# imdea-software/legosnark

Measured on AMD Instinct MI355X. Metric: alt_bn128 G1 MSM point-scalar pairs/s at n=2^20, higher is better.
Workload: dtype u32 limbs (254-bit Montgomery integers)

## Files before the change

legosnark_amd/csrc/curves.h:

```cpp
#pragma once
#include "ec.h"
#include "fp29.h"
#include "fp29x2.h"
#include "quad29.h"

namespace lsa {

struct CurveG1 {
    using Field = Fq;
    using Base = AffPacked;
    using Acc = XYZZ29;
    static constexpr bool GLV = true;
    static __device__ __forceinline__ Acc inf() { return Acc::inf(); }
    static __device__ __forceinline__ Acc madd(const Acc &a, const Base &b, bool negate, bool endo) {
        Aff29 q = unpack_affine(b);
        if (q.is_inf()) return a;
        if (negate) q.y = sub_k<1>(F29::zero(), q.y);
        if (endo) {
            constexpr uint32_t BETA29[9] = {0x0a337995u, 0x158d1d23u, 0x189c9b98u, 0x12fa4e45u, 0x185faadcu,
                                            0x0176f16du, 0x0eed93bau, 0x14291140u, 0x000c0afeu};
            q.x = mul(q.x, F29::from_limbs(BETA29));
        }
        return xyzz29_madd(a, q);
    }
    static __device__ __forceinline__ Acc add(const Acc &a, const Acc &b) { return xyzz29_add(a, b); }
    static __device__ __forceinline__ Acc dbl(const Acc &a) { return xyzz29_dbl(a); }
    static __device__ __forceinline__ Jac<Fq> to_jac(const Acc &a) { return xyzz29_to_jac(a); }
    static __device__ __forceinline__ Acc from_jac(const Jac<Fq> &p) {
        if (p.Z.is_zero()) return Acc::inf();
        F29 z = F29::from_mont256(p.Z), zz = sqr(z);
        return {F29::from_mont256(p.X), F29::from_mont256(p.Y), zz, mul(zz, z)};
    }
    static __device__ __forceinline__ Base from_affine(const Aff<Fq> &a) {
        Base r;
        if (a.is_inf()) {
#pragma unroll
            for (int i = 0; i < 8; i++) { r.x[i] = 0; r.y[i] = 0; }
        } else {
            F29::from_mont256(a.x).canonical().pack256(r.x);
            F29::from_mont256(a.y).canonical().pack256(r.y);
        }
        return r;
    }
};
struct CurveG2 {
    using Field = Fq2;
    using Base = AffPackedG2;
    using Acc = XYZZ29x2;
    static constexpr bool GLV = false;
    static __device__ __forceinline__ Acc inf() { return Acc::inf(); }
    static __device__ __forceinline__ Acc madd(const Acc &a, const Base &b, bool negate, bool ) {
        Aff29x2 q = unpack_affine(b);
        if (q.is_inf()) return a;
        if (negate) q.y = sub_k<1>(F29x2::zero(), q.y);
        return g2_madd(a, q);
    }
    static __device__ __forceinline__ Acc add(const Acc &a, const Acc &b) { return g2_add(a, b); }
    static __device__ __forceinline__ Acc dbl(const Acc &a) { return g2_dbl(a); }
    static __device__ __forceinline__ Jac<Fq2> to_jac(const Acc &a) { return g2_to_jac(a); }
    static __device__ __forceinline__ Acc from_jac(const Jac<Fq2> &p) {
        if (p.Z.is_zero()) return Acc::inf();
        F29x2 z = f29x2_from_mont256(p.Z), zz = sqr<2>(z);
        return {f29x2_from_mont256(p.X), f29x2_from_mont256(p.Y), zz, mul<2>(zz, z)};
    }
    static __device__ __forceinline__ Base from_affine(const Aff<Fq2> &a) { return pack_affine_g2(a); }
};
template <class F> struct CurveOf;
template <> struct CurveOf<Fq> { using type = CurveG1; };
template <> struct CurveOf<Fq2> { using type = CurveG2; };


}
```

legosnark_amd/csrc/fp29.h:

```cpp
#pragma once
#include "ec.h"

namespace lsa {

LSA_HD uint32_t lsa_mask(uint32_t m) {
#if defined(__HIP_DEVICE_COMPILE__)
    asm volatile("" : "+v"(m));
#endif
    return m;
}

struct F29 {
    static constexpr int W = 29;
    static constexpr uint32_t MASK = (1u << 29) - 1;
    static constexpr uint32_t PINV = 0x04866389u;
    static constexpr uint32_t PINV_POS = 0x1b799c77u;
    uint32_t l[9];

    static LSA_HD uint32_t p(int i) {
        constexpr uint32_t P29[9] = {0x187cfd47u, 0x010460b6u, 0x1c72a34fu, 0x02d522d0u, 0x1585d978u,
                                     0x02db40c0u, 0x00a6e141u, 0x0e5c2634u, 0x0030644eu};
        return P29[i];
    }
    static LSA_HD F29 from_limbs(const uint32_t (&c)[9]) {
// ... 32 lines not shown
        r.l[8] = (uint32_t)((int32_t)l[8] + c);
        return r;
    }

    friend LSA_HD F29 add_lazy(const F29 &a, const F29 &b) {
        F29 r;
#pragma unroll
        for (int i = 0; i < 9; i++) r.l[i] = a.l[i] + b.l[i];
        return r;
    }
    template <int K>
    friend LSA_HD F29 sub_k(const F29 &a, const F29 &b);

    static LSA_HD F29 redc_cols(uint64_t (&col)[17]) {
        uint64_t carry = 0;
        F29 r;
#pragma unroll
        for (int k = 0; k < 9; k++) {
            uint64_t acc = col[k] + carry;
            const uint32_t m = ((uint32_t)acc * PINV) & MASK;
            acc += (uint64_t)m * p(0);
            carry = acc >> 29;
#pragma unroll
            for (int j = 1; j < 9; j++) col[k + j] += (uint64_t)m * p(j);
        }
#pragma unroll
        for (int k = 9; k < 17; k++) {
            const uint64_t acc = col[k] + carry;
            r.l[k - 9] = (uint32_t)acc & MASK;
            carry = acc >> 29;
        }
        r.l[8] = (uint32_t)carry;
        return r;
    }
    friend LSA_HD F29 mul(const F29 &a, const F29 &b) {
#if defined(LSA_FP29_COLS)
        {
            uint64_t col[17];
#pragma unroll
            for (int k = 0; k < 17; k++) col[k] = 0;
#pragma unroll
            for (int i = 0; i < 9; i++)
#pragma unroll
                for (int j = 0; j < 9; j++) col[i + j] += (uint64_t)a.l[i] * b.l[j];
            return redc_cols(col);
        }
#endif
        uint64_t acc = 0;
        uint32_t m[9];
        F29 r;
#pragma unroll
        for (int k = 0; k < 9; k++) {
#pragma unroll
            for (int i = 0; i <= k; i++) acc += (uint64_t)a.l[i] * b.l[k - i];
#pragma unroll
            for (int i = 0; i < k; i++) acc += (uint64_t)m[i] * p(k - i);
            m[k] = ((uint32_t)acc * PINV) & MASK;
            acc += (uint64_t)m[k] * p(0);
            acc >>= 29;
        }
#pragma unroll
        for (int k = 9; k < 17; k++) {
#pragma unroll
            for (int i = k - 8; i < 9; i++) acc += (uint64_t)a.l[i] * b.l[k - i];
#pragma unroll
            for (int i = k - 8; i < 9; i++) acc += (uint64_t)m[i] * p(k - i);
            r.l[k - 9] = (uint32_t)acc & MASK;
            acc >>= 29;
        }
        r.l[8] = (uint32_t)acc;
        return r;
    }
    friend LSA_HD F29 sqr(const F29 &a) {
        uint32_t d[9];
#pragma unroll
        for (int i = 0; i < 9; i++) d[i] = a.l[i] << 1;
#if defined(LSA_FP29_COLS)
        {
            uint64_t col[17];
#pragma unroll
            for (int k = 0; k < 17; k++) col[k] = 0;
#pragma unroll
            for (int i = 0; i < 9; i++) {
                col[2 * i] += (uint64_t)a.l[i] * a.l[i];
#pragma unroll
                for (int j = i + 1; j < 9; j++) col[i + j] += (uint64_t)a.l[i] * d[j];
            }
            return redc_cols(col);
        }
#endif
        uint64_t acc = 0;
        uint32_t m[9];
        F29 r;
#pragma unroll
        for (int k = 0; k < 17; k++) {
#pragma unroll
            for (int i = 0; i < 9; i++) {
                const int j = k - i;
                if (j > i && j < 9) acc += (uint64_t)a.l[i] * d[j];
            }
            if ((k & 1) == 0) acc += (uint64_t)a.l[k / 2] * a.l[k / 2];
            if (k < 9) {
#pragma unroll
                for (int i = 0; i < k; i++) acc += (uint64_t)m[i] * p(k - i);
                m[k] = ((uint32_t)acc * PINV) & MASK;
                acc += (uint64_t)m[k] * p(0);
            } else {
#pragma unroll
                for (int i = k - 8; i < 9; i++) acc += (uint64_t)m[i] * p(k - i);
                r.l[k - 9] = (uint32_t)acc & MASK;
            }
            acc >>= 29;
        }
        r.l[8] = (uint32_t)acc;
        return r;
    }
    friend LSA_HD F29 dot2(const F29 &a0, const F29 &b0, const F29 &a1, const F29 &b1) {
#if defined(LSA_FP29_COLS)
        {
            uint64_t col[17];
#pragma unroll
            for (int k = 0; k < 17; k++) col[k] = 0;
#pragma unroll
            for (int i = 0; i < 9; i++)
#pragma unroll
                for (int j = 0; j < 9; j++) { col[i + j] += (uint64_t)a0.l[i] * b0.l[j]; col[i + j] += (uint64_t)a1.l[i] * b1.l[j]; }
            return redc_cols(col);
        }
#endif
        uint64_t acc = 0;
        uint32_t m[9];
        F29 r;
#pragma unroll
        for (int k = 0; k < 9; k++) {
#pragma unroll
            for (int i = 0; i <= k; i++) {
                acc += (uint64_t)a0.l[i] * b0.l[k - i];
                acc += (uint64_t)a1.l[i] * b1.l[k - i];
            }
#pragma unroll
            for (int i = 0; i < k; i++) acc += (uint64_t)m[i] * p(k - i);
            m[k] = ((uint32_t)acc * PINV) & MASK;
            acc += (uint64_t)m[k] * p(0);
            acc >>= 29;
        }
#pragma unroll
        for (int k = 9; k < 17; k++) {
#pragma unroll
            for (int i = k - 8; i < 9; i++) {
                acc += (uint64_t)a0.l[i] * b0.l[k - i];
                acc += (uint64_t)a1.l[i] * b1.l[k - i];
            }
#pragma unroll
            for (int i = k - 8; i < 9; i++) acc += (uint64_t)m[i] * p(k - i);
            r.l[k - 9] = (uint32_t)acc & MASK;
            acc >>= 29;
        }
        r.l[8] = (uint32_t)acc;
        return r;
    }

    friend LSA_HD F29 dot4(const F29 &a0, const F29 &b0, const F29 &a1, const F29 &b1, const F29 &a2, const F29 &b2, const F29 &a3, const F29 &b3) {
        uint64_t acc = 0;
        uint32_t m[9];
        F29 r;
#pragma unroll
        for (int k = 0; k < 9; k++) {
#pragma unroll
            for (int i = 0; i <= k; i++) {
                acc += (uint64_t)a0.l[i] * b0.l[k - i];
                acc += (uint64_t)a1.l[i] * b1.l[k - i];
                acc += (uint64_t)a2.l[i] * b2.l[k - i];
                acc += (uint64_t)a3.l[i] * b3.l[k - i];
            }
#pragma unroll
            for (int i = 0; i < k; i++) acc += (uint64_t)m[i] * p(k - i);
            m[k] = ((uint32_t)acc * PINV) & MASK;
            acc += (uint64_t)m[k] * p(0);
            acc >>= 29;
        }
#pragma unroll
        for (int k = 9; k < 17; k++) {
#pragma unroll
            for (int i = k - 8; i < 9; i++) {
                acc += (uint64_t)a0.l[i] * b0.l[k - i];
                acc += (uint64_t)a1.l[i] * b1.l[k - i];
                acc += (uint64_t)a2.l[i] * b2.l[k - i];
                acc += (uint64_t)a3.l[i] * b3.l[k - i];
            }
#pragma unroll
            for (int i = k - 8; i < 9; i++) acc += (uint64_t)m[i] * p(k - i);
            r.l[k - 9] = (uint32_t)acc & MASK;
            acc >>= 29;
        }
        r.l[8] = (uint32_t)acc;
        return r;
    }
    friend LSA_HD F29 lin2(const F29 &u, int cu, const F29 &v, int cv, int K) {
        F29 r;
        int64_t c = 0;
#pragma unroll
        for (int i = 0; i < 9; i++) {
#if defined(__HIP_DEVICE_COMPILE__)
            int64_t t = c;
            asm("v_mad_i64_i32 %0, vcc, %1, %2, %0" : "+v"(t) : "v"(K), "v"((int32_t)p(i)) : "vcc");
            asm("v_mad_i64_i32 %0, vcc, %1, %2, %0" : "+v"(t) : "v"(cu), "v"((int32_t)u.l[i]) : "vcc");
            asm("v_mad_i64_i32 %0, vcc, %1, %2, %0" : "+v"(t) : "v"(cv), "v"((int32_t)v.l[i]) : "vcc");
#else
            const int64_t t = (int64_t)cu * (int64_t)u.l[i] + (int64_t)cv * (int64_t)v.l[i] + (int64_t)K * (int64_t)p(i) + c;
#endif
            if (i < 8) { r.l[i] = (uint32_t)t & MASK; c = t >> 29; }
            else r.l[i] = (uint32_t)t;
        }
        return r;
    }

    LSA_HD bool is_zero_mod_p() const {
        uint32_t k = (l[0] * PINV_POS) & MASK;
        if (k >= 16) return false;
        uint64_t c = 0;
        bool eq = true;
#pragma unroll
        for (int i = 0; i < 9; i++) {
            c += (uint64_t)k * p(i);
            uint32_t want = (i < 8) ? ((uint32_t)c & MASK) : (uint32_t)c;
            eq = eq && (want == l[i]);
            c >>= 29;
        }
        return eq;
    }

    LSA_HD F29 canonical() const {
        F29 t = *this;
#pragma unroll
        for (int s = 3; s >= 0; s--) {
            F29 d;
            int32_t c = 0;
            uint64_t pc = 0;
#pragma unroll
            for (int i = 0; i < 9; i++) {
                pc += (uint64_t)p(i) << s;
                uint32_t pl = (i < 8) ? ((uint32_t)pc & MASK) : (uint32_t)pc;
                pc >>= 29;
                int32_t v = (int32_t)t.l[i] - (int32_t)pl + c;
                if (i < 8) { d.l[i] = (uint32_t)v & MASK; c = v >> 29; }
                else d.l[i] = (uint32_t)v;
            }
            bool neg = ((int32_t)d.l[8]) < 0;
#pragma unroll
            for (int i = 0; i < 9; i++) t.l[i] = neg ? t.l[i] : d.l[i];
        }
        return t;
    }

    static LSA_HD F29 unpack256(const uint32_t w[8]) {
        F29 r;
#pragma unroll
        for (int i = 0; i < 9; i++) {
            const int bit = 29 * i, j = bit >> 5, s = bit & 31;
            uint64_t two = (uint64_t)w[j] | ((uint64_t)(j + 1 < 8 ? w[j + 1] : 0) << 32);
            r.l[i] = (uint32_t)(two >> s) & MASK;
        }
        return r;
    }
    LSA_HD void pack256(uint32_t w[8]) const {
#pragma unroll
        for (int j = 0; j < 8; j++) w[j] = 0;
#pragma unroll
        for (int i = 0; i < 9; i++) {
            const int bit = 29 * i, j = bit >> 5, s = bit & 31;
            uint64_t v = (uint64_t)l[i] << s;
            w[j] |= (uint32_t)v;
            if (j + 1 < 8) w[j + 1] |= (uint32_t)(v >> 32);
        }
    }
    static LSA_HD F29 from_mont256(const Fq &v) {
        constexpr uint32_t C[9] = {0x13349ca1u, 0x1a5d84a8u, 0x0a3e5cacu, 0x100249e0u, 0x12b951e8u,
                                   0x0e92d304u, 0x14cb95b3u, 0x041b9d3du, 0x00058003u};
        return mul(unpack256(v.l), from_limbs(C));
    }
    LSA_HD Fq to_mont256() const {
        constexpr uint32_t D[9] = {0x058f0d9du, 0x1aea1c6eu, 0x11c2cf74u, 0x11d651ebu, 0x1462c0a7u,
                                   0x11b7bc3cu, 0x1cbd99bau, 0x183340fbu, 0x000e0a77u};
        F29 t = mul(*this, from_limbs(D)).canonical();
        Fq r;
        t.pack256(r.l);
        return r;
    }
};

template <int K>
LSA_HD F29 sub_k(const F29 &a, const F29 &b) {
    F29 r;
    uint64_t pc = 0;
    int32_t c = 0;
#pragma unroll
    for (int i = 0; i < 9; i++) {
        pc += (uint64_t)F29::p(i) * (uint32_t)K;
        uint32_t kp = (i < 8) ? ((uint32_t)pc & F29::MASK) : (uint32_t)pc;
        pc >>= 29;
        int32_t v = (int32_t)a.l[i] + (int32_t)kp - (int32_t)b.l[i] + c;
        if (i < 8) { r.l[i] = (uint32_t)v & F29::MASK; c = v >> 29; }
        else r.l[i] = (uint32_t)v;
    }
    return r;
}

struct Aff29 {
    F29 x, y;
    LSA_HD bool is_inf() const { return x.limbs_zero() && y.limbs_zero(); }
};
struct AffPacked {
    uint32_t x[8], y[8];
};
struct XYZZ29 {
    F29 X, Y, ZZ, ZZZ;
    LSA_HD bool is_inf() const { return ZZ.limbs_zero(); }
    static LSA_HD XYZZ29 inf() { return {F29::zero(), F29::zero(), F29::zero(), F29::zero()}; }
};

LSA_HD Aff29 unpack_affine(const AffPacked &q) { return {F29::unpack256(q.x), F29::unpack256(q.y)}; }

LSA_HD XYZZ29 xyzz29_dbl_affine(const Aff29 &b) {
    F29 U = add_lazy(b.y, b.y);
    F29 V = sqr(U);
    F29 W = mul(U, V);
    F29 S = mul(b.x, V);
    F29 xx = sqr(b.x);
    F29 M = add_lazy(add_lazy(xx, xx), xx).norm();
    F29 X3 = sub_k<4>(sqr(M), add_lazy(S, S));
    F29 Y3 = dot2(M, sub_k<8>(S, X3), W, sub_k<1>(F29::zero(), b.y));
    return {X3, Y3, V, W};
}

LSA_HD XYZZ29 xyzz29_dbl(const XYZZ29 &a) {
    if (a.is_inf()) return a;
    F29 U = add_lazy(a.Y, a.Y);
    F29 V = sqr(U);
    F29 W = mul(U, V);
    F29 S = mul(a.X, V);
    F29 xx = sqr(a.X);
    F29 M = add_lazy(add_lazy(xx, xx), xx).norm();
    F29 X3 = sub_k<4>(sqr(M), add_lazy(S, S));
    F29 Y3 = dot2(M, sub_k<8>(S, X3), W, sub_k<4>(F29::zero(), a.Y));
    return {X3, Y3, mul(V, a.ZZ), mul(W, a.ZZZ)};
}

LSA_HD XYZZ29 xyzz29_madd(const XYZZ29 &a, const Aff29 &b) {
    if (b.is_inf()) return a;
    if (a.is_inf()) return {b.x, b.y, F29::one(), F29::one()};
    F29 U2 = mul(b.x, a.ZZ);
    F29 S2 = mul(b.y, a.ZZZ);
    F29 Pd = sub_k<8>(U2, a.X);
    F29 R = sub_k<4>(S2, a.Y);
    if (Pd.is_zero_mod_p()) {
        if (R.is_zero_mod_p()) return xyzz29_dbl_affine(b);
        return XYZZ29::inf();
    }
    F29 PP = sqr(Pd);
    F29 PPP = mul(Pd, PP);
    F29 Q = mul(a.X, PP);
    F29 X3 = sub_k<6>(sqr(R), add_lazy(PPP, add_lazy(Q, Q)));
    F29 Y3 = dot2(R, sub_k<8>(Q, X3), sub_k<4>(F29::zero(), a.Y), PPP);
    return {X3, Y3, mul(a.ZZ, PP), mul(a.ZZZ, PPP)};
}

LSA_HD XYZZ29 xyzz29_add(const XYZZ29 &a, const XYZZ29 &b) {
    if (b.is_inf()) return a;
    if (a.is_inf()) return b;
    F29 U1 = mul(a.X, b.ZZ);
    F29 U2 = mul(b.X, a.ZZ);
    F29 S1 = mul(a.Y, b.ZZZ);
    F29 S2 = mul(b.Y, a.ZZZ);
    F29 Pd = sub_k<2>(U2, U1);
    F29 R = sub_k<2>(S2, S1);
    if (Pd.is_zero_mod_p()) {
        if (R.is_zero_mod_p()) return xyzz29_dbl(a);
        return XYZZ29::inf();
    }
    F29 PP = sqr(Pd);
    F29 PPP = mul(Pd, PP);
    F29 Q = mul(U1, PP);
    F29 X3 = sub_k<6>(sqr(R), add_lazy(PPP, add_lazy(Q, Q)));
    F29 Y3 = dot2(R, sub_k<8>(Q, X3), sub_k<2>(F29::zero(), S1), PPP);
    return {X3, Y3, mul(mul(a.ZZ, b.ZZ), PP), mul(mul(a.ZZZ, b.ZZZ), PPP)};
}

LSA_HD XYZZ29 xyzz29_neg(const XYZZ29 &a) {
    if (a.is_inf()) return a;
    return {a.X, sub_k<4>(F29::zero(), a.Y), a.ZZ, a.ZZZ};
}

LSA_HD Jac<Fq> xyzz29_to_jac(const XYZZ29 &a) {
    if (a.is_inf()) return Jac<Fq>::inf();
    F29 Xj = mul(a.X, sqr(a.ZZ));
    F29 Yj = mul(a.Y, sqr(a.ZZZ));
    return {Xj.to_mont256(), Yj.to_mont256(), a.ZZZ.to_mont256()};
}

}
```

legosnark_amd/csrc/msm.hip:

```cpp
#include <hip/hip_runtime.h>
#include <stdint.h>
#include <stdio.h>
#include <stdlib.h>
#include <string.h>
#include <algorithm>
#include <type_traits>
#include <vector>

#include "curves.h"
#include "fp29x2l.h"
#include "fs29.h"
#include "glv.h"
#include "msm.h"
#include "msm_plan.h"

namespace lsa {

unsigned msm_window_bits(size_t n) {
    unsigned lg = 0;
    while ((size_t(1) << (lg + 1)) <= n) lg++;
    int c = (int)lg - 4;
    if (c < 8) c = 8;
    if (c > 16) c = 16;
    return (unsigned)c;
// ... 457 lines not shown
}
#define PART_TILE 2048u
#define PART_SEGS 768u
#define PART_STAGE 28672u
__global__ __launch_bounds__(1024) void k_partition(const Fr *__restrict__ scalars, size_t n, SegList segs, WidePlan pl, uint32_t B, uint32_t Bc,
                                                    CoarseMap cm, uint32_t pitch, const uint16_t *__restrict__ tile_hist,
                                                    const uint32_t *__restrict__ hist_c, uint32_t *__restrict__ offs_c,
                                                    const uint32_t *__restrict__ tile_base, uint32_t *__restrict__ recs) {
    __builtin_amdgcn_s_setprio(3);
    extern __shared__ __attribute__((aligned(16))) uint32_t stage[];
    __shared__ uint32_t lstart[PART_SEGS + 1], lcur[PART_SEGS], gdst[PART_SEGS], wtot[2][PART_SEGS / 64];
    const uint32_t t = xcd_tile(blockIdx.x, gridDim.x);
    const unsigned lane = threadIdx.x & 63, wv = threadIdx.x >> 6;
    {
        uint32_t gv = 0, lv = 0;
        if (threadIdx.x < Bc) { gv = hist_c[threadIdx.x]; lv = tile_hist[(size_t)t * pitch + threadIdx.x]; }
        uint32_t gi = gv, li = lv;
#pragma unroll
        for (int d = 1; d < 64; d <<= 1) {
            const uint32_t a = __shfl_up(gi, d, 64), b = __shfl_up(li, d, 64);
            if ((int)lane >= d) { gi += a; li += b; }
        }
        if (wv < PART_SEGS / 64 && lane == 63) { wtot[0][wv] = gi; wtot[1][wv] = li; }
        __syncthreads();
        if (threadIdx.x < Bc) {
            uint32_t gex = gi - gv, lex = li - lv;
            for (unsigned w = 0; w < wv; w++) { gex += wtot[0][w]; lex += wtot[1][w]; }
            lstart[threadIdx.x] = lex;
            lcur[threadIdx.x] = lex;
            gdst[threadIdx.x] = gex + tile_base[(size_t)t * pitch + threadIdx.x];
            if (blockIdx.x == 0) offs_c[threadIdx.x] = gex;
            if (threadIdx.x == Bc - 1) lstart[Bc] = lex + lv;
        }
    }
    __syncthreads();
    const size_t lo = (size_t)t * PART_TILE;
    const uint32_t fine_bits = cm.sh_hi;
    const uint32_t tlow = t & ((1u << (16 - fine_bits)) - 1);
    for (uint32_t j = 0; j < PART_TILE / 1024; j++) {
        const uint32_t il = threadIdx.x + j * 1024;
        const size_t i = lo + il;
        if (i >= n) break;
        const uint32_t seg = segment_of(segs, (uint32_t)i);
        wide_digits(scalars[i], pl, seg * B, [&](unsigned k, int32_t sd) {
            if (sd != 0) {
                const uint32_t b = (uint32_t)(sd < 0 ? -sd : sd) - 1;
                const uint32_t pos = atomicAdd(&lcur[cm.bin(b)], 1u);
                stage[pos] = (tlow << (16 + fine_bits)) | (cm.fine(b) << 16) | (k << 12) | (sd < 0 ? 0x800u : 0u) | il;
            }
        });
    }
    __syncthreads();
    for (uint32_t sg = threadIdx.x >> 5; sg < Bc; sg += 32) {
        const uint32_t a = lstart[sg], e = lstart[sg + 1], g = gdst[sg];
        for (uint32_t x = a + (lane & 31); x < e; x += 32) recs[g + (x - a)] = stage[x];
    }
}

__global__ __launch_bounds__(1024) void k_fine_sort_part(const uint32_t *__restrict__ recs, const uint32_t *__restrict__ offs_c,
                                                         const uint32_t *__restrict__ hist_c, const uint32_t *__restrict__ tile_base,
                                                         uint32_t pitch, uint32_t T, CoarseMap cm, SegList segs, uint32_t win_stride, uint32_t stage_cap,
                                                         uint32_t *__restrict__ entries, uint32_t *__restrict__ hist, uint32_t *__restrict__ offs) {
    __builtin_amdgcn_s_setprio(3);
    extern __shared__ __attribute__((aligned(16))) uint32_t sm[];
    __shared__ uint32_t wsum[16];
    const uint32_t sg = blockIdx.x, lo = offs_c[sg], ns = hist_c[sg];
    const uint32_t fine_bits = cm.sh_hi, FM = 1u << fine_bits, fmask = FM - 1, tbits = 16 - fine_bits;
    const uint32_t F = 1u << cm.bits(sg), bucket0 = cm.first(sg);
    uint32_t *cnt = sm, *cur = sm + FM, *col = sm + 2 * FM, *stage = col + T + 1;
    const unsigned lane = threadIdx.x & 63, wv = threadIdx.x >> 6;
    for (uint32_t x = threadIdx.x; x < F; x += 1024) cnt[x] = 0;
    for (uint32_t x = threadIdx.x; x < T; x += 1024) col[x] = tile_base[(size_t)x * pitch + sg];
    if (threadIdx.x == 0) col[T] = ns;
    auto scan_counters = [&]() {
        const uint32_t per = (F + 1023) >> 10, f0 = threadIdx.x * per;
        uint32_t sum = 0;
        for (uint32_t q = 0; q < per; q++) if (f0 + q < F) sum += cnt[f0 + q];
        uint32_t incl = sum;
#pragma unroll
        for (int d = 1; d < 64; d <<= 1) {
            const uint32_t u = __shfl_up(incl, d, 64);
            if ((int)lane >= d) incl += u;
        }
        if (lane == 63) wsum[wv] = incl;
        __syncthreads();
        uint32_t run = incl - sum;
        for (unsigned w = 0; w < wv; w++) run += wsum[w];
        for (uint32_t q = 0; q < per; q++) {
            if (f0 + q >= F) break;
            const uint32_t c = cnt[f0 + q];
            cur[f0 + q] = run;
            hist[(size_t)bucket0 + f0 + q] = c;
            offs[(size_t)bucket0 + f0 + q] = lo + run;
            run += c;
        }
    };
    auto entry_of = [&](uint32_t r, uint32_t p2) {
        uint32_t a = 0, e = (T + (1u << tbits) - 1) >> tbits;
        while (e - a > 1) {
            const uint32_t m = (a + e) >> 1;
            if (col[m << tbits] <= p2) a = m; else e = m;
        }
        const uint32_t i = ((a << tbits) | (r >> (16 + fine_bits))) * PART_TILE + (r & 0x7ffu);
        const uint32_t local = i - segs.off[segment_of(segs, i)];
        return (local + ((r >> 12) & 15u) * win_stride) | ((r & 0x800u) << 20);
    };
    if (ns <= stage_cap) {
        constexpr uint32_t NR = PART_STAGE / 1024;
        uint32_t r[NR];
#pragma unroll
        for (uint32_t u = 0; u < NR; u++) { const uint32_t p2 = threadIdx.x + u * 1024; r[u] = p2 < ns ? recs[lo + p2] : 0u; }
        __syncthreads();
        uint16_t rk[NR];
#pragma unroll
        for (uint32_t u = 0; u < NR; u++) {
            rk[u] = 0;
            if (threadIdx.x + u * 1024 < ns) rk[u] = (uint16_t)atomicAdd(&cnt[(r[u] >> 16) & fmask], 1u);
        }
        __syncthreads();
        scan_counters();
        __syncthreads();
#pragma unroll
        for (uint32_t u = 0; u < NR; u++) {
            const uint32_t p2 = threadIdx.x + u * 1024;
            if (p2 < ns) stage[cur[(r[u] >> 16) & fmask] + rk[u]] = entry_of(r[u], p2);
        }
        __syncthreads();
        for (uint32_t x = threadIdx.x; x < ns; x += 1024) entries[lo + x] = stage[x];
        return;
    }
    __syncthreads();
    constexpr uint32_t UNR = 8;
    for (uint32_t p0 = threadIdx.x; p0 < ns; p0 += 1024 * UNR) {
        uint32_t r[UNR];
#pragma unroll
        for (uint32_t u = 0; u < UNR; u++) { const uint32_t p2 = p0 + u * 1024; r[u] = p2 < ns ? recs[lo + p2] : 0u; }
#pragma unroll
        for (uint32_t u = 0; u < UNR; u++) if (p0 + u * 1024 < ns) (void)lds_inc_rank(cnt, (r[u] >> 16) & fmask);
    }
    __syncthreads();
    scan_counters();
    __syncthreads();
    for (uint32_t p0 = threadIdx.x; p0 < ns; p0 += 1024 * UNR) {
        uint32_t r[UNR];
#pragma unroll
        for (uint32_t u = 0; u < UNR; u++) { const uint32_t p2 = p0 + u * 1024; r[u] = p2 < ns ? recs[lo + p2] : 0u; }
#pragma unroll
        for (uint32_t u = 0; u < UNR; u++) {
            const uint32_t p2 = p0 + u * 1024;
            if (p2 >= ns) break;
            entries[lo + lds_inc_rank(cur, (r[u] >> 16) & fmask)] = entry_of(r[u], p2);
        }
    }
}

template <class Rec>
struct RecOps;
template <>
struct RecOps<uint64_t> {
    static constexpr uint32_t NF = 128;
    static __device__ __forceinline__ uint32_t fine(uint64_t r) { return (uint32_t)(r >> 32); }
    static __device__ __forceinline__ uint32_t entry(uint64_t r) { return (uint32_t)r; }
};
template <>
struct RecOps<uint32_t> {
    static constexpr uint32_t NF = 64;
    static __device__ __forceinline__ uint32_t fine(uint32_t r) { return (r >> 25) & 63u; }
    static __device__ __forceinline__ uint32_t entry(uint32_t r) { return r & 0x81ffffffu; }
};
template <class Rec>
__global__ __launch_bounds__(1024) void k_fine_sort(const Rec *__restrict__ recs, const uint32_t *__restrict__ offs_c,
                                                    const uint32_t *__restrict__ hist_c, uint32_t *__restrict__ entries,
                                                    uint32_t *__restrict__ hist, uint32_t *__restrict__ offs) {
    using O = RecOps<Rec>;
    constexpr uint32_t NF = O::NF;
    __shared__ uint32_t cnt[NF], cur[NF];
    const uint32_t bin = blockIdx.x, lo = offs_c[bin], n = hist_c[bin];
    if (threadIdx.x < NF) cnt[threadIdx.x] = 0;
    __syncthreads();
    for (uint32_t j = threadIdx.x; j < n; j += 1024) atomicAdd(&cnt[O::fine(recs[lo + j])], 1u);
    __syncthreads();
    if (threadIdx.x < 64) {
        constexpr uint32_t PER = NF / 64;
        uint32_t c[PER], tot = 0;
#pragma unroll
        for (uint32_t q = 0; q < PER; q++) { c[q] = cnt[PER * threadIdx.x + q]; tot += c[q]; }
        uint32_t incl = tot;
#pragma unroll
        for (int d = 1; d < 64; d <<= 1) {
            uint32_t t = __shfl_up(incl, d, 64);
            if ((int)threadIdx.x >= d) incl += t;
        }
        uint32_t ex = incl - tot;
#pragma unroll
        for (uint32_t q = 0; q < PER; q++) {
            cur[PER * threadIdx.x + q] = ex;
            hist[(size_t)bin * NF + PER * threadIdx.x + q] = c[q];
            offs[(size_t)bin * NF + PER * threadIdx.x + q] = lo + ex;
            ex += c[q];
        }
    }
    __syncthreads();
    for (uint32_t j = threadIdx.x; j < n; j += 1024) {
        const Rec r = recs[lo + j];
        const uint32_t pos = atomicAdd(&cur[O::fine(r)], 1u);
        entries[lo + pos] = O::entry(r);
    }
}

#define SIZE_BINS 1025
__device__ __forceinline__ uint32_t size_bin(uint32_t cnt, uint32_t bin_shift) { return ((cnt - 1) >> bin_shift) + 1; }
template <class C>
__global__ __launch_bounds__(256) void k_size_hist(const uint32_t *__restrict__ hist, uint32_t nb, uint32_t thr, uint32_t *__restrict__ bin_count,
                                                   uint32_t group_size, uint32_t bin_shift) {
    bin_count += (group_size ? (blockIdx.x * 2048u) / group_size : 0u) * SIZE_BINS;
    __shared__ uint32_t lcnt[SIZE_BINS];
    for (uint32_t t = threadIdx.x; t < SIZE_BINS; t += 256) lcnt[t] = 0;
    __syncthreads();
    const uint32_t base = blockIdx.x * 2048 + threadIdx.x;
#pragma unroll
    for (int j = 0; j < 8; j++) {
        uint32_t g = base + j * 256;
        if (g < nb) { uint32_t cnt = hist[g]; if (cnt > 0 && cnt <= thr) atomicAdd(&lcnt[size_bin(cnt, bin_shift)], 1u); }
    }
    __syncthreads();
    for (uint32_t t = threadIdx.x; t < SIZE_BINS; t += 256) if (lcnt[t]) atomicAdd(&bin_count[t], lcnt[t]);
}
__global__ __launch_bounds__(256) void k_size_scan(const uint32_t *__restrict__ bin_count, uint32_t *__restrict__ bin_start, uint32_t ngroups) {
    __shared__ uint32_t lds[4];
    uint32_t carry = 0;
    for (uint32_t gidx = 0; gidx < ngroups; gidx++) {
        const uint32_t *bc = bin_count + gidx * SIZE_BINS;
        uint32_t *bs = bin_start + gidx * SIZE_BINS;
        uint32_t v[4], s = 0;
#pragma unroll
        for (int j = 0; j < 4; j++) {
            int bin = (int)SIZE_BINS - 1 - (int)(threadIdx.x * 4 + j);
            v[j] = (bin >= 1) ? bc[bin] : 0;
            s += v[j];
        }
        uint32_t tot;
        uint32_t run = carry + block_exclusive_scan_256(s, lds, &tot);
#pragma unroll
        for (int j = 0; j < 4; j++) {
            int bin = (int)SIZE_BINS - 1 - (int)(threadIdx.x * 4 + j);
            if (bin >= 1) bs[bin] = run;
            run += v[j];
        }
        carry += tot;
    }
    if (threadIdx.x == 0) bin_start[0] = carry;
}
template <class C>
__global__ __launch_bounds__(256) void k_size_scatter(const uint32_t *__restrict__ hist, uint32_t nb, uint32_t thr, const uint32_t *__restrict__ bin_start,
                                                      uint32_t *__restrict__ bin_cursor, uint32_t *__restrict__ perm,
                                                      uint32_t *__restrict__ heavy_list, uint32_t *__restrict__ heavy_count,
                                                      typename C::Acc *__restrict__ buckets, uint32_t group_size, uint32_t bin_shift,
                                                      uint32_t split) {
    const uint32_t goff = (group_size ? (blockIdx.x * 2048u) / group_size : 0u) * SIZE_BINS;
    bin_start += goff;
    bin_cursor += goff;
    __shared__ uint32_t lcnt[SIZE_BINS];
    for (uint32_t t = threadIdx.x; t < SIZE_BINS; t += 256) lcnt[t] = 0;
    __syncthreads();
    const uint32_t base = blockIdx.x * 2048 + threadIdx.x;
    uint32_t cnt[8], rank[8];
#pragma unroll
    for (int j = 0; j < 8; j++) {
        uint32_t g = base + j * 256;
        cnt[j] = 0; rank[j] = 0;
        if (g < nb) {
            cnt[j] = hist[g];
            if (cnt[j] == 0) { for (uint32_t h = 0; h < split; h++) buckets[(size_t)g * split + h] = C::inf(); }
            else if (cnt[j] > thr) heavy_list[atomicAdd(heavy_count, 1u)] = g;
            else rank[j] = atomicAdd(&lcnt[size_bin(cnt[j], bin_shift)], 1u);
        }
    }
    __syncthreads();
    for (uint32_t t = threadIdx.x; t < SIZE_BINS; t += 256) {
        uint32_t c = lcnt[t];
        lcnt[t] = c ? atomicAdd(&bin_cursor[t], c) : 0;
    }
    __syncthreads();
#pragma unroll
    for (int j = 0; j < 8; j++) {
        uint32_t g = base + j * 256;
        if (g < nb && cnt[j] > 0 && cnt[j] <= thr) {
            const uint32_t bin = size_bin(cnt[j], bin_shift);
            perm[bin_start[bin] + lcnt[bin] + rank[j]] = g;
        }
    }
}

template <class C, uint32_t ACC_SPLIT>
__device__ __forceinline__ void accumulate_body(const typename C::Base *__restrict__ bases, const uint32_t *__restrict__ entries,
                                                const uint32_t *__restrict__ offs, const uint32_t *__restrict__ hist,
                                                const uint32_t *__restrict__ perm, const uint32_t *__restrict__ nperm,
                                                typename C::Acc *__restrict__ buckets) {
    uint32_t t = blockIdx.x * blockDim.x + threadIdx.x;
    if (t >= *nperm * ACC_SPLIT) return;
    const uint32_t g = perm[t / ACC_SPLIT], part = t % ACC_SPLIT;
    const uint32_t cnt = hist[g];
    const uint32_t *e = entries + offs[g];
    typename C::Acc acc = C::inf();
    if (part < cnt) {
        uint32_t v = e[part];
        typename C::Base cur = bases[v & 0x3fffffffu];
        for (uint32_t j = part; j < cnt; j += ACC_SPLIT) {
            uint32_t vn = v;
            typename C::Base nxt = cur;
            if (j + ACC_SPLIT < cnt) { vn = e[j + ACC_SPLIT]; nxt = bases[vn & 0x3fffffffu]; }
            acc = C::madd(acc, cur, (v >> 31) != 0, ((v >> 30) & 1) != 0);
            v = vn;
            cur = nxt;
        }
    }
    buckets[(size_t)g * ACC_SPLIT + part] = acc;
}
template <class C, uint32_t ACC_SPLIT>
__global__ __launch_bounds__(256) void k_accumulate(const typename C::Base *__restrict__ bases, const uint32_t *__restrict__ entries,
                                                    const uint32_t *__restrict__ offs, const uint32_t *__restrict__ hist,
                                                    const uint32_t *__restrict__ perm, const uint32_t *__restrict__ nperm,
                                                    typename C::Acc *__restrict__ buckets) {
    accumulate_body<C, ACC_SPLIT>(bases, entries, offs, hist, perm, nperm, buckets);
}
__global__ __launch_bounds__(256) __attribute__((amdgpu_waves_per_eu(2, 2))) void k_accumulate_g2_occ2(
    const CurveG2::Base *__restrict__ bases, const uint32_t *__restrict__ entries, const uint32_t *__restrict__ offs,
    const uint32_t *__restrict__ hist, const uint32_t *__restrict__ perm, const uint32_t *__restrict__ nperm, CurveG2::Acc *__restrict__ buckets) {
    accumulate_body<CurveG2, 1u>(bases, entries, offs, hist, perm, nperm, buckets);
}

__global__ __launch_bounds__(256) void k_accumulate_g2_pair(const AffPackedG2 *__restrict__ bases, const uint32_t *__restrict__ entries,
                                                            const uint32_t *__restrict__ offs, const uint32_t *__restrict__ hist,
                                                            const uint32_t *__restrict__ perm, const uint32_t *__restrict__ nperm,
                                                            XYZZ29x2 *__restrict__ buckets) {
    const uint32_t t = blockIdx.x * blockDim.x + threadIdx.x, pr = t >> 1, part = t & 1;
    if (pr >= *nperm) return;
    const uint32_t g = perm[pr];
    const uint32_t cnt = hist[g];
    const uint32_t *e = entries + offs[g];
    struct Half { uint32_t x[8], y[8]; };
    auto fetch = [&](uint32_t v) {
        const AffPackedG2 &b = bases[v & 0x3fffffffu];
        Half h;
#pragma unroll
        for (int i = 0; i < 8; i++) { h.x[i] = b.w[part][i]; h.y[i] = b.w[2 + part][i]; }
        return h;
    };
    XyzzE<F29h> acc = XyzzE<F29h>::inf();
    uint32_t v = e[0];
    Half cur = fetch(v);
    for (uint32_t j = 0; j < cnt; j++) {
        uint32_t vn = v;
        Half nxt = cur;
        if (j + 1 < cnt) { vn = e[j + 1]; nxt = fetch(vn); }
        AffE<F29h> q = {{F29::unpack256(cur.x)}, {F29::unpack256(cur.y)}};
        if (!q.is_inf()) {
            if (v >> 31) q.y = sub_k<1>(F29h::zero(), q.y);
            acc = g2_madd(acc, q);
        }
        v = vn;
        cur = nxt;
    }
    F29 *o = reinterpret_cast<F29 *>(&buckets[g]);
    o[part] = acc.X.v;
    o[2 + part] = acc.Y.v;
    o[4 + part] = acc.ZZ.v;
    o[6 + part] = acc.ZZZ.v;
}

template <class A>
__device__ __forceinline__ A shfl_down_acc(const A &p, unsigned delta) {
    A r;
    constexpr int NW = sizeof(A) / 4;
    const uint32_t *src = reinterpret_cast<const uint32_t *>(&p);
    uint32_t *dst = reinterpret_cast<uint32_t *>(&r);
#pragma unroll
    for (int i = 0; i < NW; i++) dst[i] = __shfl_down(src[i], delta, 64);
    return r;
}

template <class C>
__device__ __forceinline__ typename C::Acc wave_sum(typename C::Acc v, unsigned lane) {
    for (unsigned d = 32; d >= 1; d >>= 1) {
        typename C::Acc t = shfl_down_acc(v, d);
        if (lane + d < 64) v = C::add(v, t);
    }
    return v;
}

#define HEAVY_CHUNK 512u
__global__ __launch_bounds__(256) void k_heavy_plan(const uint32_t *__restrict__ hist, const uint32_t *__restrict__ heavy_list,
                                                    const uint32_t *__restrict__ heavy_count, uint32_t *__restrict__ chunk_off) {
    __shared__ uint32_t lds[4];
    __shared__ uint32_t s_chunk;
    const uint32_t nh = *heavy_count;
    uint32_t carry = 0;
    for (uint32_t base = 0; base < nh; base += 256) {
        uint32_t h = base + threadIdx.x;
        uint32_t tot;
        (void)block_exclusive_scan_256(h < nh ? hist[heavy_list[h]] : 0, lds, &tot);
        carry += tot;
    }
    if (threadIdx.x == 0) {
        uint32_t chunk = HEAVY_CHUNK;
        while (chunk < 4096u && carry / (2 * chunk) >= 2048u) chunk *= 2;
        s_chunk = chunk;
    }
    __syncthreads();
    const uint32_t chunk = s_chunk;
    carry = 0;
    for (uint32_t base = 0; base < nh; base += 256) {
        uint32_t h = base + threadIdx.x;
        uint32_t v = h < nh ? (hist[heavy_list[h]] + chunk - 1) / chunk : 0;
        uint32_t tot;
        uint32_t ex = block_exclusive_scan_256(v, lds, &tot);
        if (h < nh) chunk_off[h] = carry + ex;
        carry += tot;
    }
    if (threadIdx.x == 0) { chunk_off[nh] = carry; chunk_off[nh + 1] = chunk; }
}

template <class C>
__global__ __launch_bounds__(64) void k_accumulate_heavy(const typename C::Base *__restrict__ bases, const uint32_t *__restrict__ entries,
                                                         const uint32_t *__restrict__ offs, const uint32_t *__restrict__ hist,
                                                         const uint32_t *__restrict__ heavy_list, const uint32_t *__restrict__ heavy_count,
                                                         const uint32_t *__restrict__ chunk_off, typename C::Acc *__restrict__ partials) {
    const uint32_t nh = *heavy_count;
    if (nh == 0) return;
    const uint32_t total = chunk_off[nh], chunk = chunk_off[nh + 1];
    const unsigned lane = threadIdx.x;
    for (uint32_t v = blockIdx.x; v < total; v += gridDim.x) {
        uint32_t lo = 0, hi = nh;
        while (hi - lo > 1) { uint32_t mid = (lo + hi) >> 1; if (chunk_off[mid] <= v) lo = mid; else hi = mid; }
        const uint32_t g = heavy_list[lo];
        const uint32_t cnt = hist[g];
        const uint32_t start = (v - chunk_off[lo]) * chunk;
        const uint32_t end = start + chunk < cnt ? start + chunk : cnt;
        const uint32_t *e = entries + offs[g];
        typename C::Acc acc = C::inf();
        for (uint32_t j = start + lane; j < end; j += 64) {
            uint32_t w = e[j];
            acc = C::madd(acc, bases[w & 0x3fffffffu], (w >> 31) != 0, ((w >> 30) & 1) != 0);
        }
        acc = wave_sum<C>(acc, lane);
        if (lane == 0) partials[v] = acc;
    }
}

template <class C>
__global__ __launch_bounds__(64) void k_heavy_finish(const uint32_t *__restrict__ heavy_list, const uint32_t *__restrict__ heavy_count,
                                                     const uint32_t *__restrict__ chunk_off, const typename C::Acc *__restrict__ partials,
                                                     typename C::Acc *__restrict__ buckets, uint32_t split) {
    const uint32_t nh = *heavy_count;
    unsigned lane = threadIdx.x;
    for (uint32_t h = blockIdx.x; h < nh; h += gridDim.x) {
        typename C::Acc acc = C::inf();
        for (uint32_t v = chunk_off[h] + lane; v < chunk_off[h + 1]; v += 64) acc = C::add(acc, partials[v]);
        acc = wave_sum<C>(acc, lane);
        if (lane == 0) {
            buckets[(size_t)heavy_list[h] * split] = acc;
            for (uint32_t x = 1; x < split; x++) buckets[(size_t)heavy_list[h] * split + x] = C::inf();
        }
    }
}

template <class A>
__device__ __forceinline__ A select_acc(uint32_t mask, const A &a, const A &b) {
    A r;
    const uint32_t *pa = reinterpret_cast<const uint32_t *>(&a), *pb = reinterpret_cast<const uint32_t *>(&b);
    uint32_t *pr = reinterpret_cast<uint32_t *>(&r);
#pragma unroll
    for (int i = 0; i < (int)(sizeof(A) / 4); i++) pr[i] = (pa[i] & mask) | (pb[i] & ~mask);
    return r;
}
template <class A>
__device__ __forceinline__ void quadwave_weighted(A &acc, A &run, unsigned log_mult, unsigned lane) {
    const unsigned q = lane & 3, qi = lane >> 2;
    A s = A::inf();
#pragma unroll 1
    for (unsigned step = 0; step < 9; step++) {
        if (step == 4) {
            s = (qi == 0) ? A::inf() : run;
#pragma unroll 1
            for (unsigned i = 0; i < log_mult; i++) s = quad_dbl(s, q);
        }
        uint32_t m_run = step < 4 ? 0xffffffffu : 0u, m_s = step == 4 ? 0xffffffffu : 0u;
        asm volatile("" : "+v"(m_run), "+v"(m_s));
        const unsigned d = step < 4 ? (1u << step) : (step == 4 ? 0u : (8u >> (step - 5)));
        const A lhs = select_acc(m_run, run, acc);
        const A rhs = select_acc(m_s, s, shfl_down_acc(lhs, 4 * d));
        A r = lhs;
        if (qi + d < 16) r = quad_add(lhs, rhs, q);
        run = select_acc(m_run, r, run);
        acc = select_acc(m_run, acc, r);
    }
}

template <class C>
__global__ __launch_bounds__(64) void k_reduce1_lane(const typename C::Acc *__restrict__ buckets, uint32_t B, uint32_t L, uint32_t split,
                                                     typename C::Acc *__restrict__ out) {
    using A = typename C::Acc;
    const uint32_t t = blockIdx.x * 64 + threadIdx.x;
    if ((uint64_t)t * L >= B) return;
    A acc = A::inf(), run = A::inf();
    const A *bk = buckets + (size_t)t * L * split;
    const uint32_t per = split + 1;
#pragma unroll 1
    for (int i = (int)L - 1; i >= 0; i--) {
#pragma unroll 1
        for (uint32_t h = 0; h < per; h++) {
            uint32_t m = h < split ? 0xffffffffu : 0u;
            asm volatile("" : "+v"(m));
            A rhs = run;
            if (h < split) rhs = bk[(size_t)i * split + h];
            const A lhs = select_acc(m, run, acc);
            const A r = C::add(lhs, rhs);
            run = select_acc(m, r, run);
            acc = select_acc(m, acc, r);
        }
    }
    out[2 * (size_t)t] = acc;
    out[2 * (size_t)t + 1] = run;
}

template <class C>
__global__ __launch_bounds__(64) void k_reduce2_lane(const typename C::Acc *__restrict__ in, uint32_t m_in, uint32_t m_out, uint32_t log_mult,
                                                     typename C::Acc *__restrict__ out) {
    using A = typename C::Acc;
    const uint32_t t = blockIdx.x * 64 + threadIdx.x;
    if (t >= m_out) return;
    A acc = A::inf(), run = A::inf(), wsum = A::inf();
#pragma unroll 1
    for (int j = 15; j >= 0; j--) {
        const uint32_t idx = 16 * t + (uint32_t)j;
        const bool have = idx < m_in;
        const uint32_t trips = j ? 3u : 2u;
#pragma unroll 1
        for (uint32_t h = 0; h < trips; h++) {
            uint32_t m0 = h == 0 ? 0xffffffffu : 0u, m1 = h == 1 ? 0xffffffffu : 0u;
            asm volatile("" : "+v"(m0), "+v"(m1));
            A rhs = run;
            if (h < 2) rhs = have ? in[2 * (size_t)idx + h] : A::inf();
            const A lhs = select_acc(m0, acc, select_acc(m1, run, wsum));
            const A r = C::add(lhs, rhs);
            acc = select_acc(m0, r, acc);
            run = select_acc(m1, r, run);
            wsum = select_acc(~(m0 | m1), r, wsum);
        }
    }
#pragma unroll 1
    for (uint32_t i = 0; i < log_mult; i++) wsum = C::dbl(wsum);
    out[2 * (size_t)t] = C::add(acc, wsum);
    out[2 * (size_t)t + 1] = run;
}

template <class C>
__global__ __launch_bounds__(64) void k_reduce1(const typename C::Acc *__restrict__ buckets, uint32_t B, uint32_t L, uint32_t logL,
                                                uint32_t waves_per_window, uint32_t split, typename C::Acc *__restrict__ wave_out) {
    using A = typename C::Acc;
    uint32_t wave = blockIdx.x;
    uint32_t k = wave / waves_per_window, w = wave % waves_per_window;
    const unsigned lane = threadIdx.x, q = lane & 3;
    uint32_t t = w * 16 + (lane >> 2);
    A acc = A::inf(), run = A::inf();
    if ((uint64_t)t * L < B) {
        const A *bk = buckets + ((size_t)k * B + (size_t)t * L) * split;
        const uint32_t per = split + 1;
#pragma unroll 1
        for (int i = (int)L - 1; i >= 0; i--) {
#pragma unroll 1
            for (uint32_t h = 0; h < per; h++) {
                uint32_t m = h < split ? 0xffffffffu : 0u;
                asm volatile("" : "+v"(m));
                A rhs = run;
                if (h < split) rhs = bk[(size_t)i * split + h];
                const A lhs = select_acc(m, run, acc);
                const A r = quad_add(lhs, rhs, q);
                run = select_acc(m, r, run);
                acc = select_acc(m, acc, r);
            }
        }
    }
    quadwave_weighted(acc, run, logL, lane);
    if (lane == 0) {
        wave_out[2 * (size_t)wave] = acc;
        wave_out[2 * (size_t)wave + 1] = run;
    }
}

template <class C>
__global__ __launch_bounds__(64) void k_reduce2(const typename C::Acc *__restrict__ in, uint32_t m_in, uint32_t m_out, uint32_t log_mult,
                                                typename C::Acc *__restrict__ out) {
    using A = typename C::Acc;
    const uint32_t k = blockIdx.x / m_out, w = blockIdx.x % m_out;
    const unsigned lane = threadIdx.x;
    const uint32_t j = w * 16 + (lane >> 2);
    A acc = A::inf(), run = A::inf();
    if (j < m_in) {
        acc = in[2 * ((size_t)k * m_in + j)];
        run = in[2 * ((size_t)k * m_in + j) + 1];
    }
    quadwave_weighted(acc, run, log_mult, lane);
    if (lane == 0) {
        out[2 * ((size_t)k * m_out + w)] = acc;
        out[2 * ((size_t)k * m_out + w) + 1] = run;
    }
}

template <class A>
__device__ __forceinline__ void pin_vgpr(A &a) {
    uint32_t *w = reinterpret_cast<uint32_t *>(&a);
#pragma unroll
    for (int i = 0; i < (int)(sizeof(A) / 4); i++) asm volatile("" : "+v"(w[i]));
}
// ... 783 lines not shown
```

Measured before the change: 768.9 million.

## Specialize G1 bucket accumulation with affine head add and signed madd

In bucket accumulation for G1, the first two affine points are now combined with a dedicated affine+affine add, which avoids the multiplications by ZZ=ZZZ=1 in the first mixed add. Negation is folded into the R subtraction through a mask (sub_k_signed), and some subtractions use a loose non-normalizing form. The endomorphism multiply is compiled out when ACC_SPLIT is 1. Together these cut field multiplications and branching per bucket, at the cost of more code size and register pressure. Correctness for the rare equal-x cases now depends on the new helper path.

After: 794.0 million, median of 6. 3.3% higher.

```diff
diff --git a/legosnark_amd/csrc/curves.h b/legosnark_amd/csrc/curves.h
--- a/legosnark_amd/csrc/curves.h
+++ b/legosnark_amd/csrc/curves.h
@@ -12,16 +12,15 @@
     using Acc = XYZZ29;
     static constexpr bool GLV = true;
     static __device__ __forceinline__ Acc inf() { return Acc::inf(); }
+    template <bool ENDO = true>
     static __device__ __forceinline__ Acc madd(const Acc &a, const Base &b, bool negate, bool endo) {
-        Aff29 q = unpack_affine(b);
-        if (q.is_inf()) return a;
-        if (negate) q.y = sub_k<1>(F29::zero(), q.y);
-        if (endo) {
-            constexpr uint32_t BETA29[9] = {0x0a337995u, 0x158d1d23u, 0x189c9b98u, 0x12fa4e45u, 0x185faadcu,
-                                            0x0176f16du, 0x0eed93bau, 0x14291140u, 0x000c0afeu};
-            q.x = mul(q.x, F29::from_limbs(BETA29));
-        }
-        return xyzz29_madd(a, q);
+        return g1_madd_packed<ENDO>(a, b, negate, endo);
+    }
+    static constexpr bool HEAD = true;
+    static __device__ __forceinline__ bool head_ok(const Base &b0, const Base &b1) { return !packed_is_inf(b0) && !packed_is_inf(b1); }
+    template <bool ENDO = true>
+    static __device__ __forceinline__ Acc madd_head(const Base &b0, bool neg0, bool endo0, const Base &b1, bool neg1, bool endo1) {
+        return g1_madd_head<ENDO>(b0, neg0, endo0, b1, neg1, endo1);
     }
     static __device__ __forceinline__ Acc add(const Acc &a, const Acc &b) { return xyzz29_add(a, b); }
     static __device__ __forceinline__ Acc dbl(const Acc &a) { return xyzz29_dbl(a); }
@@ -49,6 +48,8 @@
     using Acc = XYZZ29x2;
     static constexpr bool GLV = false;
     static __device__ __forceinline__ Acc inf() { return Acc::inf(); }
+    static constexpr bool HEAD = false;
+    template <bool ENDO = true>
     static __device__ __forceinline__ Acc madd(const Acc &a, const Base &b, bool negate, bool ) {
         Aff29x2 q = unpack_affine(b);
         if (q.is_inf()) return a;
diff --git a/legosnark_amd/csrc/fp29.h b/legosnark_amd/csrc/fp29.h
--- a/legosnark_amd/csrc/fp29.h
+++ b/legosnark_amd/csrc/fp29.h
@@ -358,6 +358,39 @@
         int32_t v = (int32_t)a.l[i] + (int32_t)kp - (int32_t)b.l[i] + c;
         if (i < 8) { r.l[i] = (uint32_t)v & F29::MASK; c = v >> 29; }
         else r.l[i] = (uint32_t)v;
+    }
+    return r;
+}
+
+template <int K>
+LSA_HD F29 sub_k_signed(const F29 &s, const F29 &b, uint32_t m) {
+    F29 r;
+    uint64_t pc = 0;
+    const uint32_t m29 = m & F29::MASK;
+    int32_t c = (int32_t)(m & 1u);
+#pragma unroll
+    for (int i = 0; i < 9; i++) {
+        pc += (uint64_t)F29::p(i) * (uint32_t)K;
+        uint32_t kp = (i < 8) ? ((uint32_t)pc & F29::MASK) : (uint32_t)pc;
+        pc >>= 29;
+        int32_t v = (int32_t)(s.l[i] ^ (i < 8 ? m29 : m)) + (int32_t)kp - (int32_t)b.l[i] + c;
+        if (i < 8) { r.l[i] = (uint32_t)v & F29::MASK; c = v >> 29; }
+        else r.l[i] = (uint32_t)v;
+    }
+    return r;
+}
+
+template <int K>
+LSA_HD F29 sub_loose(const F29 &a, const F29 &b) {
+    F29 r;
+    uint64_t pc = 0;
+#pragma unroll
+    for (int i = 0; i < 9; i++) {
+        pc += (uint64_t)F29::p(i) * (uint32_t)K;
+        const uint32_t kp = (i < 8) ? ((uint32_t)pc & F29::MASK) : (uint32_t)pc;
+        pc >>= 29;
+        const uint32_t c = (i == 0) ? kp + (1u << 29) : (i < 8) ? kp + F29::MASK : kp - 1u;
+        r.l[i] = a.l[i] + c - b.l[i];
     }
     return r;
 }
@@ -421,6 +454,44 @@
     return {X3, Y3, mul(a.ZZ, PP), mul(a.ZZZ, PPP)};
 }
 
+LSA_HD XYZZ29 xyzz29_madd_rare(const XYZZ29 &a, const Aff29 &b, uint32_t m, const F29 &R) {
+    Aff29 q = b;
+    if (m) q.y = sub_k<1>(F29::zero(), b.y);
+    if (a.is_inf()) return {q.x, q.y, F29::one(), F29::one()};
+    if (R.is_zero_mod_p()) return xyzz29_dbl_affine(q);
+    return XYZZ29::inf();
+}
+LSA_HD XYZZ29 xyzz29_madd_signed(const XYZZ29 &a, const Aff29 &b, uint32_t m) {
+    F29 U2 = mul(b.x, a.ZZ);
+    F29 S2 = mul(b.y, a.ZZZ);
+    F29 Pd = sub_k<8>(U2, a.X);
+    F29 R = sub_k_signed<6>(S2, a.Y, m);
+    if (Pd.is_zero_mod_p()) return xyzz29_madd_rare(a, b, m, R);
+    F29 PP = sqr(Pd);
+    F29 PPP = mul(Pd, PP);
+    F29 Q = mul(a.X, PP);
+    F29 X3 = sub_k<6>(sqr(R), add_lazy(PPP, add_lazy(Q, Q)));
+    F29 Y3 = dot2(R, sub_loose<10>(Q, X3), sub_loose<6>(F29::zero(), a.Y), PPP);
+    return {X3, Y3, mul(a.ZZ, PP), mul(a.ZZZ, PPP)};
+}
+
+LSA_HD XYZZ29 xyzz29_add_affine(const Aff29 &a, const Aff29 &b, uint32_t m) {
+    F29 Pd = sub_k<2>(b.x, a.x);
+    F29 R = sub_k_signed<2>(b.y, a.y, m);
+    if (Pd.is_zero_mod_p()) {
+        if (!R.is_zero_mod_p()) return XYZZ29::inf();
+        Aff29 q = b;
+        if (m) q.y = sub_k<1>(F29::zero(), b.y);
+        return xyzz29_dbl_affine(q);
+    }
+    F29 PP = sqr(Pd);
+    F29 PPP = mul(Pd, PP);
+    F29 Q = mul(a.x, PP);
+    F29 X3 = sub_k<6>(sqr(R), add_lazy(PPP, add_lazy(Q, Q)));
+    F29 Y3 = dot2(R, sub_loose<10>(Q, X3), sub_loose<3>(F29::zero(), a.y), PPP);
+    return {X3, Y3, PP, PPP};
+}
+
 LSA_HD XYZZ29 xyzz29_add(const XYZZ29 &a, const XYZZ29 &b) {
     if (b.is_inf()) return a;
     if (a.is_inf()) return b;
@@ -442,6 +513,35 @@
     return {X3, Y3, mul(mul(a.ZZ, b.ZZ), PP), mul(mul(a.ZZZ, b.ZZZ), PPP)};
 }
 
+LSA_HD bool packed_is_inf(const AffPacked &q) {
+    if ((q.x[0] | q.y[0]) != 0) return false;
+    uint32_t o = 0;
+#pragma unroll
+    for (int i = 1; i < 8; i++) o |= q.x[i] | q.y[i];
+    return o == 0;
+}
+template <bool ENDO>
+LSA_HD Aff29 g1_unpack_base(const AffPacked &b, bool endo) {
+    Aff29 q = unpack_affine(b);
+    if (ENDO && endo) {
+        constexpr uint32_t BETA29[9] = {0x0a337995u, 0x158d1d23u, 0x189c9b98u, 0x12fa4e45u, 0x185faadcu,
+                                        0x0176f16du, 0x0eed93bau, 0x14291140u, 0x000c0afeu};
+        q.x = mul(q.x, F29::from_limbs(BETA29));
+    }
+    return q;
+}
+template <bool ENDO>
+LSA_HD XYZZ29 g1_madd_packed(const XYZZ29 &a, const AffPacked &b, bool negate, bool endo) {
+    if (packed_is_inf(b)) return a;
+    return xyzz29_madd_signed(a, g1_unpack_base<ENDO>(b, endo), lsa_mask(negate ? ~0u : 0u));
+}
+template <bool ENDO>
+LSA_HD XYZZ29 g1_madd_head(const AffPacked &b0, bool neg0, bool endo0, const AffPacked &b1, bool neg1, bool endo1) {
+    Aff29 q0 = g1_unpack_base<ENDO>(b0, endo0);
+    if (neg0) q0.y = sub_k<1>(F29::zero(), q0.y);
+    return xyzz29_add_affine(q0, g1_unpack_base<ENDO>(b1, endo1), lsa_mask(neg1 ? ~0u : 0u));
+}
+
 LSA_HD XYZZ29 xyzz29_neg(const XYZZ29 &a) {
     if (a.is_inf()) return a;
     return {a.X, sub_k<4>(F29::zero(), a.Y), a.ZZ, a.ZZZ};
diff --git a/legosnark_amd/csrc/msm.hip b/legosnark_amd/csrc/msm.hip
--- a/legosnark_amd/csrc/msm.hip
+++ b/legosnark_amd/csrc/msm.hip
@@ -783,15 +783,32 @@
     const uint32_t g = perm[t / ACC_SPLIT], part = t % ACC_SPLIT;
     const uint32_t cnt = hist[g];
     const uint32_t *e = entries + offs[g];
+    constexpr bool ENDO = ACC_SPLIT != 1;
     typename C::Acc acc = C::inf();
     if (part < cnt) {
         uint32_t v = e[part];
         typename C::Base cur = bases[v & 0x3fffffffu];
-        for (uint32_t j = part; j < cnt; j += ACC_SPLIT) {
+        uint32_t j = part;
+        if constexpr (C::HEAD) {
+            if (j + ACC_SPLIT < cnt) {
+                const uint32_t v1 = e[j + ACC_SPLIT];
+                const typename C::Base b1 = bases[v1 & 0x3fffffffu];
+                if (C::head_ok(cur, b1)) {
+                    uint32_t vn = v1;
+                    typename C::Base nxt = b1;
+                    if (j + 2 * ACC_SPLIT < cnt) { vn = e[j + 2 * ACC_SPLIT]; nxt = bases[vn & 0x3fffffffu]; }
+                    acc = C::template madd_head<ENDO>(cur, (v >> 31) != 0, ((v >> 30) & 1) != 0, b1, (v1 >> 31) != 0, ((v1 >> 30) & 1) != 0);
+                    j += 2 * ACC_SPLIT;
+                    v = vn;
+                    cur = nxt;
+                }
+            }
+        }
+        for (; j < cnt; j += ACC_SPLIT) {
             uint32_t vn = v;
             typename C::Base nxt = cur;
             if (j + ACC_SPLIT < cnt) { vn = e[j + ACC_SPLIT]; nxt = bases[vn & 0x3fffffffu]; }
-            acc = C::madd(acc, cur, (v >> 31) != 0, ((v >> 30) & 1) != 0);
+            acc = C::template madd<ENDO>(acc, cur, (v >> 31) != 0, ((v >> 30) & 1) != 0);
             v = vn;
             cur = nxt;
         }
```
